# arkCyber/whisper-rust

Measured on AMD Instinct MI355X. Metric: real-time factor (audio-sec/wall-sec), greedy, 30 s synthetic chunks, higher is better.
Workload: dtype f16 operands / f32 accumulate; 1 GPU; ggml-small-shaped synthetic F16 model, greedy best_of=1 temperature_inc=0, 1 x 30 s 16 kHz f32 chunk per GPU, PCM resident in HBM; flash_attn=False, parallelism=chunk-dp1

## Files before the change

include/whisper_amd.h:

```cpp
#ifndef WHISPER_AMD_H
#define WHISPER_AMD_H

#include <stdbool.h>
#include <stddef.h>
#include <stdint.h>

#if defined(__GNUC__)
#  define WHISPER_API __attribute__((visibility("default")))
#else
#  define WHISPER_API
#endif

#define WHISPER_SAMPLE_RATE 16000
#define WHISPER_N_FFT       400
#define WHISPER_HOP_LENGTH  160
#define WHISPER_CHUNK_SIZE  30

#ifdef __cplusplus
extern "C" {
#endif

enum ggml_log_level {
    GGML_LOG_LEVEL_NONE  = 0,
    GGML_LOG_LEVEL_DEBUG = 1,
// ... 302 lines not shown
WHISPER_API struct whisper_vad_context_params whisper_vad_default_context_params(void);
WHISPER_API struct whisper_vad_context * whisper_vad_init_from_file_with_params(const char * path_model, struct whisper_vad_context_params params);
WHISPER_API struct whisper_vad_context * whisper_vad_init_with_params          (struct whisper_model_loader * loader, struct whisper_vad_context_params params);
WHISPER_API bool    whisper_vad_detect_speech(struct whisper_vad_context * vctx, const float * samples, int n_samples);
WHISPER_API int     whisper_vad_n_probs(struct whisper_vad_context * vctx);
WHISPER_API float * whisper_vad_probs  (struct whisper_vad_context * vctx);
WHISPER_API struct whisper_vad_segments * whisper_vad_segments_from_probs  (struct whisper_vad_context * vctx, struct whisper_vad_params params);
WHISPER_API struct whisper_vad_segments * whisper_vad_segments_from_samples(struct whisper_vad_context * vctx, struct whisper_vad_params params, const float * samples, int n_samples);
WHISPER_API int   whisper_vad_segments_n_segments(struct whisper_vad_segments * segments);
WHISPER_API float whisper_vad_segments_get_segment_t0(struct whisper_vad_segments * segments, int i_segment);
WHISPER_API float whisper_vad_segments_get_segment_t1(struct whisper_vad_segments * segments, int i_segment);
WHISPER_API void  whisper_vad_free_segments(struct whisper_vad_segments * segments);
WHISPER_API void  whisper_vad_free         (struct whisper_vad_context  * ctx);

WHISPER_API int          whisper_bench_memcpy          (int n_threads);
WHISPER_API const char * whisper_bench_memcpy_str      (int n_threads);
WHISPER_API int          whisper_bench_ggml_mul_mat    (int n_threads);
WHISPER_API const char * whisper_bench_ggml_mul_mat_str(int n_threads);


WHISPER_API void whisper_amd_abi_sizes(size_t out[6]);

WHISPER_API int64_t whisper_amd_get_mel      (struct whisper_state * state, float * dst, int64_t cap, int * n_len, int * n_mel);
WHISPER_API int64_t whisper_amd_get_embd_enc (struct whisper_state * state, float * dst, int64_t cap);
WHISPER_API int64_t whisper_amd_get_embd_conv(struct whisper_state * state, float * dst, int64_t cap);

WHISPER_API int64_t whisper_amd_vad_front  (struct whisper_vad_context * vctx, const float * samples, int n_samples, float * dst, int64_t cap);
WHISPER_API int     whisper_amd_vad_tile   (void);
WHISPER_API void    whisper_amd_vad_timings(struct whisper_vad_context * vctx, int64_t out_us[3]);

WHISPER_API void whisper_amd_get_timings_us(struct whisper_state * state, int64_t out[12]);
WHISPER_API void whisper_amd_reset_timings (struct whisper_state * state);

WHISPER_API void whisper_amd_gelu_table_f16(uint16_t * dst);

WHISPER_API void * whisper_amd_state_stream(struct whisper_state * state);

WHISPER_API int whisper_amd_decoder_info(struct whisper_state * state, int j, double out[8], int32_t * ids, int max_ids);

WHISPER_API int whisper_amd_decode_step_probe(struct whisper_context * ctx, struct whisper_state * state, int n_past, int n_iters, float * ms_per_step);

WHISPER_API int whisper_amd_mega_enabled(struct whisper_state * state);
WHISPER_API void whisper_amd_mega_role_of(int n_wg, int n_head, int wg, int * role, int * index);

WHISPER_API void whisper_amd_overlap_stats(struct whisper_state * state, int out[2]);

WHISPER_API int whisper_amd_mega_debug(struct whisper_context * ctx, struct whisper_state * state, int token, int n_past,
                                       unsigned long long * granules_out, float * logits_out);
WHISPER_API int whisper_amd_seq_debug(struct whisper_context * ctx, struct whisper_state * state, int token, int n_past, unsigned * values_out,
                                      float * logits_out);

WHISPER_API void whisper_amd_rows_stats(struct whisper_state * state, long out[2]);
WHISPER_API int  whisper_amd_rows_enabled(struct whisper_state * state);
WHISPER_API int whisper_amd_rows_debug(struct whisper_context * ctx, struct whisper_state * state, int B, int token, int n_past,
                                       unsigned long long * granules_out, float * logits_out);
WHISPER_API int whisper_amd_rows_step_probe(struct whisper_context * ctx, struct whisper_state ** states, int B, int n_past, int n_iters, float * ms_per_step);

WHISPER_API int whisper_amd_full_batch(struct whisper_context * ctx, struct whisper_state ** states, int n_chunks,
                                       struct whisper_full_params params, const float * const * samples, const int * n_samples);
WHISPER_API void whisper_amd_batch_stats(struct whisper_context * ctx, long * steps, long * rows);
WHISPER_API long whisper_amd_batch_one_launch(struct whisper_context * ctx);

#ifdef __cplusplus
}
#endif
#endif
// ... 1 lines not shown
```

whisper-rust_amd/csrc/wa_api.cpp:

```cpp
#include "wa_internal.h"

#include <algorithm>
#include <chrono>
#include <cmath>
#include <cstdarg>
#include <cstring>
#include <regex>
#include <thread>

static void wa_log_default(ggml_log_level, const char * text, void *) { fputs(text, stderr); fflush(stderr); }
static ggml_log_callback g_log_cb = wa_log_default;
static void * g_log_ud = nullptr;

void wa_log(ggml_log_level level, const char * fmt, ...) {
    if (!g_log_cb) return;
    char buf[1024];
    va_list ap;
    va_start(ap, fmt);
    const int n = vsnprintf(buf, sizeof(buf), fmt, ap);
    va_end(ap);
    if (n < (int) sizeof(buf)) { g_log_cb(level, buf, g_log_ud); return; }
    std::vector<char> big(n + 1);
    va_start(ap, fmt);
    vsnprintf(big.data(), big.size(), fmt, ap);
// ... 639 lines not shown
whisper_token_data whisper_full_get_token_data(struct whisper_context * ctx, int i, int j) { return ctx->state->result_all[i].tokens[j]; }
float whisper_full_get_token_p_from_state(struct whisper_state * st, int i, int j) { return st->result_all[i].tokens[j].p; }
float whisper_full_get_token_p(struct whisper_context * ctx, int i, int j) { return ctx->state->result_all[i].tokens[j].p; }
float whisper_full_get_segment_no_speech_prob_from_state(struct whisper_state * st, int i) { return st->result_all[i].no_speech_prob; }
float whisper_full_get_segment_no_speech_prob(struct whisper_context * ctx, int i) { return ctx->state->result_all[i].no_speech_prob; }

int          whisper_bench_memcpy(int) { return 0; }
const char * whisper_bench_memcpy_str(int) { return "whisper_bench_memcpy: not applicable to the HIP backend (use bench.py)\n"; }
int          whisper_bench_ggml_mul_mat(int) { return 0; }
const char * whisper_bench_ggml_mul_mat_str(int) { return "whisper_bench_ggml_mul_mat: not applicable to the HIP backend (use bench.py)\n"; }

static int64_t copy_out(whisper_state * st, const float * d_src, int64_t n, float * dst, int64_t cap) {
    if (!d_src) return -1;
    if (dst && cap > 0) {
        (void) hipSetDevice(st->ctx->device);
        (void) hipStreamSynchronize(st->stream);
        if (hipMemcpy(dst, d_src, (size_t) std::min(n, cap) * sizeof(float), hipMemcpyDeviceToHost) != hipSuccess) return -1;
    }
    return n;
}
int64_t whisper_amd_get_mel(struct whisper_state * st, float * dst, int64_t cap, int * n_len, int * n_mel) {
    if (n_len) *n_len = st->mel_n_len;
    if (n_mel) *n_mel = st->mel_n_mel;
    return copy_out(st, st->d_mel, (int64_t) st->mel_n_len * st->mel_n_mel, dst, cap);
}
int64_t whisper_amd_get_embd_enc(struct whisper_state * st, float * dst, int64_t cap) {
    if (!st->have_enc) return -1;
    return copy_out(st, st->d_embd_enc, (int64_t) st->enc_n_ctx * st->ctx->model.hp.n_audio_state, dst, cap);
}
int64_t whisper_amd_get_embd_conv(struct whisper_state * st, float * dst, int64_t cap) {
    if (!st->have_enc) return -1;
    return copy_out(st, st->d_embd_conv, (int64_t) st->enc_n_ctx * st->ctx->model.hp.n_audio_state, dst, cap);
}
void whisper_amd_gelu_table_f16(uint16_t * dst) {
    for (int i = 0; i < 65536; ++i) {
        _Float16 h; uint16_t u = (uint16_t) i; memcpy(&h, &u, 2);
        const float x = (float) h;
        const float g = 0.5f * x * (1.0f + tanhf(0.79788456080286535587989211986876f * x * (1.0f + 0.044715f * x * x)));
        _Float16 o = (_Float16) g; memcpy(&dst[i], &o, 2);
    }
}
void * whisper_amd_state_stream(struct whisper_state * st) { return (void *) st->stream; }

int whisper_amd_decoder_info(struct whisper_state * st, int j, double out[8], int32_t * ids, int max_ids) {
    if (!st || j < 0 || j >= WA_MAX_DECODERS) return -1;
    const auto & d = st->decoders[j];
    out[0] = d.failed; out[1] = d.completed; out[2] = d.has_ts; out[3] = d.seek_delta; out[4] = d.sequence.result_len;
    out[5] = d.sequence.avg_logprobs; out[6] = d.sequence.entropy; out[7] = st->no_speech_prob;
    const int n = (int) d.sequence.tokens.size();
    for (int i = 0; i < n && i < max_ids; ++i) ids[i] = d.sequence.tokens[i].id;
    return n;
}

int whisper_amd_full_batch(struct whisper_context * ctx, struct whisper_state ** states, int n_chunks, struct whisper_full_params params,
                           const float * const * samples, const int * n_samples) {
    if (!ctx || !states || n_chunks <= 0) return -1;
    std::vector<int> rc(n_chunks, 0);
    std::vector<std::thread> th;
    th.reserve(n_chunks);
    {
        wa_batch_groups groups(ctx, std::vector<whisper_state *>(states, states + n_chunks));
        for (int i = 0; i < n_chunks; ++i)
            th.emplace_back([&, i]() {
                rc[i] = whisper_full_with_state(ctx, states[i], params, samples[i], n_samples[i]);
                wa_batcher_leave(states[i]->batcher);
            });
// ... 8 lines not shown
```

whisper-rust_amd/csrc/wa_encode.cpp:

```cpp
#include "wa_internal.h"
#include "wa_kernels.h"
#include "wa_mega.h"
#include "wa_rows.h"

#include <algorithm>
#include <cmath>
#include <cstdlib>
#include <cstring>

template <typename T> static bool dev_alloc(T *& p, size_t n_elem, bool zero = true) {
    p = nullptr;
    const size_t bytes = n_elem * sizeof(T);
    if (!WA_HIP_OK(hipMalloc((void **) &p, bytes ? bytes : 256))) return false;
    if (zero && bytes) return WA_HIP_OK(hipMemset(p, 0, bytes));
    return true;
}
template <typename T> static void dev_free(T *& p) { if (p) { (void) hipFree(p); p = nullptr; } }

bool wa_kv_self_realloc(whisper_context & ctx, whisper_state & st, int n_cells) {
    const auto & hp = ctx.model.hp;
    if (n_cells > WA_ATT_MAXKV) { WA_ERROR("%s: %d KV cells exceed the attention kernels' limit (%d)\n", __func__, n_cells, WA_ATT_MAXKV); return false; }
    if (st.dec_graph) { (void) hipGraphExecDestroy(st.dec_graph); st.dec_graph = nullptr; }
    dev_free(st.kv_self.k);
    dev_free(st.kv_self.v);
    st.kv_self.size = n_cells;
    st.kv_self.head = 0;
    st.kv_self.n = 0;
    st.kv_self.cells.assign(n_cells, wa_kv_cell());
    const size_t n = (size_t) hp.n_text_layer * n_cells * hp.n_text_state;
    if (!dev_alloc(st.kv_self.k, n) || !dev_alloc(st.kv_self.v, n)) return false;
    dev_free(st.d_mask);
    st.d_mask_cap = (size_t) st.dec_mpad * n_cells;
    if (!dev_alloc(st.d_mask, st.d_mask_cap)) return false;
    if (st.h_stage_mask) { (void) hipHostFree(st.h_stage_mask); st.h_stage_mask = nullptr; }
    st.h_mask_cap = st.d_mask_cap;
    if (!WA_HIP_OK(hipHostMalloc((void **) &st.h_stage_mask, st.h_mask_cap))) return false;
    return true;
}

bool wa_rows_prepare(whisper_context & ctx, whisper_state & st) {
    if (!st.rows_form.enabled()) return false;
    if (st.d_rows_gr) return true;
    const auto & hp = ctx.model.hp;
    const int dt = hp.n_text_state, Ht = hp.n_text_head;
    const size_t row_gr = (size_t) 2 * dt;
    if (!dev_alloc(st.d_rows_gr, (size_t) hp.n_text_layer * WA_MEGA_EDGES * WA_ROWS_MAX * row_gr) ||
        !dev_alloc(st.d_rows_cgr, (size_t) hp.n_text_layer * WA_ROWS_MAX * Ht * WA_ROWS_CGR) || !dev_alloc(st.d_rows_status, 32)) {
        dev_free(st.d_rows_gr); dev_free(st.d_rows_cgr); dev_free(st.d_rows_status);
        st.rows_form.disable();
        return false;
    }
    return true;
}

bool wa_state_alloc(whisper_context & ctx, whisper_state & st) {
    const auto & hp = ctx.model.hp;
    const int d = hp.n_audio_state;
    st.ctx = &ctx;
    if (!WA_HIP_OK(hipSetDevice(ctx.device))) return false;
    if (!WA_HIP_OK(hipStreamCreateWithFlags(&st.stream, hipStreamNonBlocking))) return false;

    const int T = hp.n_audio_ctx, tpad = wa_pad(T, WA_TPAD);
    st.enc_tpad = tpad;
    st.cross_tpad = tpad;
    if (!dev_alloc(st.d_mel_max, 1)) return false;
    if (!dev_alloc(st.d_melT, (size_t) (2 * T + 8) * hp.n_mels + 512)) return false;
    if (!dev_alloc(st.d_h1,   (size_t) (2 * T + 8) * d)) return false;
    if (!dev_alloc(st.d_x,    (size_t) tpad * d)) return false;
    if (!dev_alloc(st.d_xn,   (size_t) tpad * d)) return false;
    if (!dev_alloc(st.d_qk,   (size_t) tpad * 2 * d)) return false;
    if (!dev_alloc(st.d_vt,   (size_t) d * tpad)) return false;
    if ((ctx.exact || ctx.model.wtype != 1) && hp.n_audio_state == hp.n_audio_head * 64)
        if (!dev_alloc(st.d_attn_p, (size_t) hp.n_audio_head * tpad * tpad) || !dev_alloc(st.d_attn_pl, (size_t) hp.n_audio_head * tpad * 32)) return false;
    if (!dev_alloc(st.d_ao,   (size_t) tpad * d)) return false;
    if (!dev_alloc(st.d_ff,   (size_t) tpad * 4 * d)) return false;
    if (!dev_alloc(st.d_embd_enc,  (size_t) tpad * d)) return false;
    if (!dev_alloc(st.d_embd_conv, (size_t) tpad * d)) return false;
    const size_t n_cross = (size_t) hp.n_text_layer * hp.n_text_head * tpad * 64;
    if (!dev_alloc(st.d_cross_k, n_cross) || !dev_alloc(st.d_cross_v, n_cross)) return false;

    const int mpad = wa_pad(hp.n_text_ctx, 64);
    st.dec_mpad = mpad;
    if (!dev_alloc(st.d_tok, mpad) || !dev_alloc(st.d_pos, mpad) || !dev_alloc(st.d_cell, mpad) || !dev_alloc(st.d_rows, mpad)) return false;
    if (!dev_alloc(st.d_dx,   (size_t) mpad * d)) return false;
    if (!dev_alloc(st.d_dxn,  (size_t) mpad * d)) return false;
    if (!dev_alloc(st.d_dqkv, (size_t) mpad * 3 * d)) return false;
    if (!dev_alloc(st.d_dao,  (size_t) mpad * d)) return false;
    if (!dev_alloc(st.d_dff,  (size_t) mpad * 4 * d)) return false;
    if (!dev_alloc(st.d_dq,   (size_t) mpad * d)) return false;
    if (!dev_alloc(st.d_logits, (size_t) WA_MAX_DECODERS * hp.n_vocab + 64, false)) return false;
    if (!dev_alloc(st.d_dyn, 8)) return false;
    { const char * g = getenv("WHISPER_AMD_NO_GRAPH"); st.graphs_enabled = !(g && g[0] == '1'); }
    {
        const char * g = getenv("WHISPER_AMD_NO_MEGA");
        const int dt = hp.n_text_state, Ht = hp.n_text_head;
        st.mega_form = wa_launch_form(!(g && g[0] == '1') && ctx.model.d_mega_layers && ctx.model.n_loaded > 0 && dt == Ht * 64 && dt % 128 == 0 &&
                                      dt <= WA_MEGA_MAX_D && hp.n_audio_ctx <= 1500 && ctx.model.n_cu >= 5 * Ht + 16 && tpad <= WA_MEGA_MAX_T &&
                                      !wa_wtype_has_min(ctx.model.wtype));
        if (st.mega_form.enabled()) {
            if (!dev_alloc(st.d_mega_cgr, (size_t) hp.n_text_layer * Ht * WA_MEGA_CGR)) return false;
            if (!dev_alloc(st.d_mega_gr, (size_t) hp.n_text_layer * WA_MEGA_EDGES * 4 * dt) || !dev_alloc(st.d_mega_out, (size_t) hp.n_vocab + 64)) return false;
            st.d_mega_status = (unsigned *) (st.d_mega_out + hp.n_vocab);
            if (!dev_alloc(st.d_mega_out2, (size_t) hp.n_vocab + 64) || !dev_alloc(st.d_mega_smask, (size_t) hp.n_vocab / 32 + 2)) return false;
            for (int b = 0; b < 2; ++b)
                if (!dev_alloc(st.d_mega_rec[b], (size_t) 512 * 8) || !dev_alloc(st.d_mega_ps[b], 8)) return false;
            {
// ... 134 lines not shown
    const int tpad = st.enc_tpad;
    hipStream_t s = st.stream;
    st.enc_n_ctx = T;

    const int rows_total = 2 * T + 8;
    wa_launch_mel_window(s, st.d_mel, hp.n_mels, st.mel_n_len, mel_offset, 2 * T, st.d_melT, rows_total);

    const bool exact = ctx.exact || m.wtype != 1;
    auto gemm = [&](wa_epi_mode mode, const wa_f16 * A, int lda, const wa_f16 * W, int ldw, int M, int N, int K, const wa_epi & e) {
        if (exact) wa_launch_gemm_exact(s, mode, A, lda, W, ldw, M, N, K, e);
        else       wa_launch_gemm(s, mode, A, lda, W, ldw, M, N, K, e);
    };

    {
        wa_epi e; e.bias = m.conv1.b; e.gelu = m.d_gelu; e.out = st.d_h1 + d; e.ldo = d;
        if (exact) {
            wa_launch_im2col3(s, st.d_melT, hp.n_mels, 0, 1, hp.n_mels, 2 * T, st.d_im2col, 3 * hp.n_mels);
            wa_launch_gemm_exact(s, WA_EPI_GELU_F16, st.d_im2col, 3 * hp.n_mels, m.conv1_g, 3 * hp.n_mels, 2 * T, d, 3 * hp.n_mels, e);
        } else {
            wa_launch_gemm(s, WA_EPI_GELU_F16, st.d_melT, hp.n_mels, m.conv1.w, m.conv1_kpad, 2 * T, d, m.conv1_kpad, e);
        }
    }
    {
        wa_epi e; e.bias = m.conv2.b; e.gelu = m.d_gelu; e.out = st.d_x; e.ldo = d; e.resid = m.e_pe; e.ldr = d; e.dbg = st.d_embd_conv;
        if (exact) {
            wa_launch_im2col3(s, st.d_h1, d, 0, 2, d, T, st.d_im2col, 3 * d);
            wa_launch_gemm_exact(s, WA_EPI_CONV2, st.d_im2col, 3 * d, m.conv2_g, 3 * d, T, d, 3 * d, e);
        } else {
            wa_launch_gemm(s, WA_EPI_CONV2, st.d_h1, 2 * d, m.conv2.w, 3 * d, T, d, 3 * d, e);
        }
    }

    const float KQscale = 1.0f / sqrtf(float(64));
    if (m.wtype != 1) {
        auto qmul = [&](wa_epi_mode mode, const wa_lin & L, int M, const wa_epi & e) {
            wa_launch_qgemm_exact(s, mode, st.d_q8, st.d_q8d, M, L.qs, L.qd, L.n_out, L.n_in, e, st.d_q8s, L.qm);
        };
        auto qlin = [&](wa_epi_mode mode, const float * A, int lda, const wa_lin & L, int M, const wa_epi & e) {
            wa_launch_quantize_q8_0(s, A, lda, M, L.n_in, st.d_q8, st.d_q8d, st.d_q8s);
            qmul(mode, L, M, e);
        };
        for (int il = 0; il < hp.n_audio_layer; ++il) {
            const auto & L = m.enc[il];
            wa_launch_layernorm_exact(s, st.d_x, d, T, d, L.attn_ln.w, L.attn_ln.b, hp.eps, nullptr, 0, nullptr, 0, st.d_q8, st.d_q8d, st.d_q8s);
            static const bool no_mfma_attn = getenv("WHISPER_AMD_NO_EXACT_MFMA") != nullptr;
            if (st.d_attn_p && T >= 128 && !no_mfma_attn) {
                { wa_epi e; e.bias = L.qkv.b; e.out = st.d_qk; e.ldo = 2 * d; e.out2 = st.d_vt; e.ldo2 = tpad; e.split0 = 2 * d; qmul(WA_EPI_ENC_QKV, L.qkv, T, e); }
                wa_launch_attn_exact_mfma(s, st.d_qk, 2 * d, st.d_vt, tpad, T, d, H, KQscale, st.d_attn_p, st.d_attn_pl, (T + 127) & ~127, st.d_ao, d, st.d_q32a);
                wa_launch_quantize_q8_0(s, st.d_q32a, d, T, d, st.d_q8, st.d_q8d, st.d_q8s);
            } else {
            { wa_epi e; e.bias = L.qkv.b; e.out = st.d_ff; e.ldo = 3 * d; qmul(WA_EPI_F16, L.qkv, T, e); }
            wa_launch_attn_exact(s, st.d_ff, 3 * d, st.d_ff + d, 64, 3 * d, st.d_ff + 2 * d, 64, 3 * d, H, T, T, nullptr, KQscale,
                                 st.d_att_partial, st.d_att_pleft, st.d_ao, d, nullptr, nullptr, nullptr, wa_q8_rows{ st.d_q8, st.d_q8d, st.d_q8s });
            }
            { wa_epi e; e.bias = L.out.b; e.out = st.d_x; e.ldo = d; e.resid = st.d_x; e.ldr = d; qmul(WA_EPI_RESID, L.out, T, e); }
            wa_launch_layernorm_exact(s, st.d_x, d, T, d, L.mlp_ln.w, L.mlp_ln.b, hp.eps, nullptr, 0, nullptr, 0, st.d_q8, st.d_q8d, st.d_q8s);
            { wa_epi e; e.bias = L.fc1.b; e.gelu = m.d_gelu; e.out = st.d_q32b; e.ldo = 4 * d; qmul(WA_EPI_GELU_F32, L.fc1, T, e); }
            { wa_epi e; e.bias = L.fc2.b; e.out = st.d_x; e.ldo = d; e.resid = st.d_x; e.ldr = d; qlin(WA_EPI_RESID, st.d_q32b, 4 * d, L.fc2, T, e); }
        }
        wa_launch_layernorm_exact(s, st.d_x, d, T, d, m.e_ln.w, m.e_ln.b, hp.eps, nullptr, 0, st.d_embd_enc, d);
        {
            wa_epi e; e.bias = m.cross_kv.b; e.scale = m.cross_kv.s; e.out = st.d_cross_k; e.out2 = st.d_cross_v; e.aux0 = st.cross_tpad; e.aux1 = d;
            qlin(WA_EPI_CROSS_KV, st.d_embd_enc, d, m.cross_kv, T, e);
        }
    } else {
    for (int il = 0; il < hp.n_audio_layer; ++il) {
        const auto & L = m.enc[il];
        if (exact) wa_launch_layernorm_exact(s, st.d_x, d, T, d, L.attn_ln.w, L.attn_ln.b, hp.eps, st.d_xn, d, nullptr, 0);
        else       wa_launch_layernorm(s, st.d_x, d, T, d, L.attn_ln.w, L.attn_ln.b, hp.eps, st.d_xn, d, nullptr, 0);
        static const bool no_mfma_attn = getenv("WHISPER_AMD_NO_EXACT_MFMA") != nullptr;
        if (exact && st.d_attn_p && T >= 128 && !no_mfma_attn) {
            wa_epi e; e.bias = L.qkv.b; e.out = st.d_qk; e.ldo = 2 * d; e.out2 = st.d_vt; e.ldo2 = tpad; e.split0 = 2 * d;
            wa_launch_gemm_exact(s, WA_EPI_ENC_QKV, st.d_xn, d, L.qkv.w, d, T, 3 * d, d, e);
            wa_launch_attn_exact_mfma(s, st.d_qk, 2 * d, st.d_vt, tpad, T, d, H, KQscale, st.d_attn_p, st.d_attn_pl, (T + 127) & ~127, st.d_ao, d);
        } else if (exact) {
            wa_epi e; e.bias = L.qkv.b; e.out = st.d_ff; e.ldo = 3 * d;
            wa_launch_gemm_exact(s, WA_EPI_F16, st.d_xn, d, L.qkv.w, d, T, 3 * d, d, e);
            wa_launch_attn_exact(s, st.d_ff, 3 * d, st.d_ff + d, 64, 3 * d, st.d_ff + 2 * d, 64, 3 * d, H, T, T, nullptr, KQscale,
                                 st.d_att_partial, st.d_att_pleft, st.d_ao, d, nullptr);
        } else {
            wa_epi e; e.bias = L.qkv.b; e.out = st.d_qk; e.ldo = 2 * d; e.out2 = st.d_vt; e.ldo2 = tpad; e.split0 = 2 * d;
            wa_launch_gemm(s, WA_EPI_ENC_QKV, st.d_xn, d, L.qkv.w, d, T, 3 * d, d, e);
            wa_launch_enc_attn(s, st.d_qk, 2 * d, st.d_vt, tpad, T, d, H, KQscale, st.d_ao, d);
        }
        {
            wa_epi e; e.bias = L.out.b; e.out = st.d_x; e.ldo = d; e.resid = st.d_x; e.ldr = d;
            gemm(WA_EPI_RESID, st.d_ao, d, L.out.w, d, T, d, d, e);
        }
        if (exact) wa_launch_layernorm_exact(s, st.d_x, d, T, d, L.mlp_ln.w, L.mlp_ln.b, hp.eps, st.d_xn, d, nullptr, 0);
        else       wa_launch_layernorm(s, st.d_x, d, T, d, L.mlp_ln.w, L.mlp_ln.b, hp.eps, st.d_xn, d, nullptr, 0);
        {
            wa_epi e; e.bias = L.fc1.b; e.gelu = m.d_gelu; e.out = st.d_ff; e.ldo = 4 * d;
            gemm(WA_EPI_GELU_F16, st.d_xn, d, L.fc1.w, d, T, 4 * d, d, e);
        }
        {
            wa_epi e; e.bias = L.fc2.b; e.out = st.d_x; e.ldo = d; e.resid = st.d_x; e.ldr = d;
            gemm(WA_EPI_RESID, st.d_ff, 4 * d, L.fc2.w, 4 * d, T, d, 4 * d, e);
        }
    }
    if (exact) wa_launch_layernorm_exact(s, st.d_x, d, T, d, m.e_ln.w, m.e_ln.b, hp.eps, st.d_xn, d, st.d_embd_enc, d);
    else       wa_launch_layernorm(s, st.d_x, d, T, d, m.e_ln.w, m.e_ln.b, hp.eps, st.d_xn, d, st.d_embd_enc, d);

    {
        wa_epi e; e.bias = m.cross_kv.b; e.scale = m.cross_kv.s; e.out = st.d_cross_k; e.out2 = st.d_cross_v; e.aux0 = st.cross_tpad; e.aux1 = d;
        gemm(WA_EPI_CROSS_KV, st.d_xn, d, m.cross_kv.w, d, T, hp.n_text_layer * 2 * d, d, e);
    }
    }
// ... 7 lines not shown
```

whisper-rust_amd/csrc/wa_exact.hip:

```cpp
#include "wa_device.h"
#include <cstdlib>

#define EX_LD 40

template <int EPI>
__global__ __launch_bounds__(256, 2) void k_gemm_exact(const wa_f16 * __restrict__ A, int lda, const wa_f16 * __restrict__ W, int ldw,
                                                       int M, int N, int K, wa_epi e) {
    __shared__ __attribute__((aligned(16))) wa_f16 As[2][32 * EX_LD];
    __shared__ __attribute__((aligned(16))) wa_f16 Ws[2][32 * EX_LD];
    const int tid = threadIdx.x, lane = tid & 63, wave = tid >> 6;
    const int wm = wave >> 1, wn = wave & 1, li = lane >> 3, lj = lane & 7;
    const int tiles_n = (N + 31) / 32;
    const int m0 = (blockIdx.x / tiles_n) * 32, n0 = (blockIdx.x % tiles_n) * 32;

    float acc[2][2][32];
#pragma unroll
    for (int p = 0; p < 2; ++p)
#pragma unroll
        for (int q = 0; q < 2; ++q)
#pragma unroll
            for (int i = 0; i < 32; ++i) acc[p][q][i] = 0.0f;

    const int np = K & ~31, nsteps = np >> 5;
    const int lrow = (tid & 127) >> 2, lkc = tid & 3;
// ... 893 lines not shown
    float inv;
    {
        const double delta = 2.0 * (double) (ng + 8) * 0x1p-53 * tot * 1.000001;
        const float ilo = (float) (1.0 / (tot + delta)), ihi = (float) (1.0 / (tot - delta));
        inv = ilo;
        if (ilo != ihi) {
            double sum = 0.0;
            if (u == 0) {
                for (int g = 0; g < ng; ++g) { const float * v = srow + 8 * g; sum += (double) (((v[0] + v[4]) + (v[2] + v[6])) + ((v[1] + v[5]) + (v[3] + v[7]))); }
                for (int c = n8; c < T; ++c) sum += (double) srow[c];
            }
            sum = __shfl(sum, lane & ~31, WAVE);
            inv = (float) (1.0 / sum);
        }
    }
    if (jq >= T) return;
    wa_f16 * prow = P + ((size_t) h * T + jq) * kvp;
    wa_f16 * plrow = p_left + ((size_t) h * T + jq) * 32;
    typedef unsigned as_u4 __attribute__((ext_vector_type(4)));
    for (int g = u; g < (kvp >> 3); g += LPR) {
        as_u4 pk = { 0u, 0u, 0u, 0u };
        const int c0 = 8 * g;
        if (c0 < np) {
            const float4 lo = *(const float4 *) (srow + c0), hi = *(const float4 *) (srow + c0 + 4);
            pk.x = (unsigned) f2h(lo.x * inv) | ((unsigned) f2h(lo.y * inv) << 16); pk.y = (unsigned) f2h(lo.z * inv) | ((unsigned) f2h(lo.w * inv) << 16);
            pk.z = (unsigned) f2h(hi.x * inv) | ((unsigned) f2h(hi.y * inv) << 16); pk.w = (unsigned) f2h(hi.z * inv) | ((unsigned) f2h(hi.w * inv) << 16);
        } else {
            for (int c = c0; c < c0 + 8 && c < T; ++c) plrow[c - np] = f2h(srow[c] * inv);
        }
        *(as_u4 *) (prow + c0) = pk;
    }
}

void wa_launch_attn_exact_mfma(hipStream_t s, const wa_f16 * qk, int ldqk, const wa_f16 * vt, int ldvt, int T, int d, int n_head, float scale,
                               wa_f16 * p, wa_f16 * p_left, int kvp, wa_f16 * out, int ldo, float * out32) {
    static bool attr_done = false;
    const int lds = AS_Q * (kvp + AS_PAD) * (int) sizeof(float);
    if (!attr_done) { (void) hipFuncSetAttribute((const void *) k_attn_scores_mfma, hipFuncAttributeMaxDynamicSharedMemorySize, 160 * 1024 - 4096); attr_done = true; }
    hipLaunchKernelGGL(k_attn_scores_mfma, dim3(n_head, (T + AS_Q - 1) / AS_Q), dim3(AS_THREADS), lds, s, qk, ldqk, d, T, scale, p, p_left, kvp);
    const int np = T & ~31;
    wa_epi e; e.out = out; e.ldo = ldo; e.out2 = p_left; e.bs_o2 = (long long) T * 32; e.aux0 = np; e.aux1 = T - np;
    e.out3 = out32; e.ldo3 = ldo;
    e.bs_a = (long long) T * kvp; e.bs_w = (long long) 64 * ldvt;
    gemm_exact_mfma_launch<WA_EPI_ATTN_PV>(s, p, kvp, vt, ldvt, T, 64, (np + 127) & ~127, e, n_head);
}

template <int NQ>
__global__ __launch_bounds__(ATT_THREADS) void k_attn_exact_mq(const wa_f16 * __restrict__ q, int ldq, const wa_f16 * __restrict__ kbase, size_t k_head_stride,
                                                               int k_row_stride, const wa_f16 * __restrict__ vbase, size_t v_head_stride, int v_row_stride,
                                                               int n_tokens, int n_kv, int kvp, const int8_t * __restrict__ mask, float scale,
                                                               wa_f16 * __restrict__ out, int ldo, float * __restrict__ qk_out,
                                                               float * __restrict__ out32, int8_t * __restrict__ q8, float * __restrict__ q8d, float * __restrict__ q8s) {
    constexpr int NW = ATT_THREADS / 64;
    extern __shared__ __attribute__((aligned(16))) unsigned char mq_smem[];
    float  * sc   = (float *) mq_smem;
    float  * gs   = sc + (size_t) NQ * kvp;
    float  * part = gs + (size_t) NQ * (kvp >> 3);
    wa_f16 * p16  = (wa_f16 *) (part + (size_t) NQ * 32 * 64);
    __shared__ float red[NQ][NW];
    __shared__ double redd[NQ][NW];
    __shared__ float s_inv[NQ];
    __shared__ __attribute__((aligned(16))) wa_f16 qs[NQ][64];

    const int tid = threadIdx.x, lane = tid & 63, wave = tid >> 6;
    const int n_head = gridDim.x;
    const int h = blockIdx.x, j0 = blockIdx.y * NQ;
    const wa_f16 * kp = kbase + (size_t) h * k_head_stride;
    const wa_f16 * vp = vbase + (size_t) h * v_head_stride;
// ... 225 lines not shown
```

whisper-rust_amd/csrc/wa_internal.h:

```cpp
#pragma once

#include "../../include/whisper_amd.h"
#include "wa_one_launch.h"
#include "wa_grammar.h"
#include "wa_vad.h"

#include <hip/hip_runtime.h>

#include <cstdint>
#include <cstdio>
#include <map>
#include <memory>
#include <mutex>
#include <random>
#include <set>
#include <string>
#include <atomic>
#include <vector>

#define WA_MAX_DECODERS 8
#define WA_TPAD         128

void wa_log(ggml_log_level level, const char * fmt, ...) __attribute__((format(printf, 2, 3)));
#define WA_INFO(...)  wa_log(GGML_LOG_LEVEL_INFO,  __VA_ARGS__)
// ... 137 lines not shown
};

struct wa_decoder {
    wa_sequence sequence;
    int  i_batch = 0, seek_delta = 0;
    bool failed = false, completed = false, has_ts = false;
    std::vector<float> probs, logits, logprobs;
    std::vector<std::pair<double, int>> logits_id;
    mutable std::mt19937 rng;
    wa_grammar_state grammar;
    wa_grammar_cache grammar_cache;
};

struct whisper_state {
    whisper_context * ctx = nullptr;
    hipStream_t stream = nullptr;

    int64_t t_sample_us = 0, t_encode_us = 0, t_decode_us = 0, t_batchd_us = 0, t_prompt_us = 0, t_mel_us = 0;
    int32_t n_sample = 0, n_encode = 0, n_decode = 0, n_batchd = 0, n_prompt = 0, n_fail_p = 0, n_fail_h = 0;

    int mel_n_len = 0, mel_n_len_org = 0, mel_n_mel = 0;
    float * d_mel = nullptr; size_t d_mel_cap = 0;
    float * d_pcm = nullptr; size_t d_pcm_cap = 0;
    unsigned int * d_mel_max = nullptr;

    int enc_n_ctx = 0;
    int enc_tpad  = 0;
    wa_f16 * d_melT   = nullptr;
    wa_f16 * d_h1     = nullptr;
    float  * d_x      = nullptr;
    wa_f16 * d_xn     = nullptr;
    wa_f16 * d_qk     = nullptr;
    wa_f16 * d_vt     = nullptr;
    wa_f16 * d_attn_p = nullptr;
    wa_f16 * d_attn_pl = nullptr;
    wa_f16 * d_ao     = nullptr;
    wa_f16 * d_ff     = nullptr;
    float  * d_embd_enc  = nullptr;
    float  * d_embd_conv = nullptr;
    bool     have_enc = false;

    wa_f16 * d_cross_k = nullptr, * d_cross_v = nullptr;
    int cross_tpad = 0;

    wa_kv_cache kv_self;
    int kv_self_n_dec = 0;

    int dec_mpad = 0;
    int32_t * d_tok = nullptr, * d_pos = nullptr, * d_cell = nullptr;
    int8_t  * d_mask = nullptr; size_t d_mask_cap = 0;
    float  * d_dx  = nullptr;
    wa_f16 * d_dxn = nullptr;
    wa_f16 * d_dqkv = nullptr;
    wa_f16 * d_dao = nullptr;
    wa_f16 * d_dff = nullptr;
    wa_f16 * d_dq  = nullptr;
    float  * d_att_partial = nullptr;
    wa_f16 * d_att_pleft = nullptr;
    wa_f16 * d_im2col = nullptr;
    float  * d_logits = nullptr;
    int32_t * d_rows = nullptr;
    float  * d_aheads_qk = nullptr;
    float  * d_q32a = nullptr;
    float  * d_q32b = nullptr;
    int8_t * d_q8   = nullptr;
    int      q8_rows = 0;
    float  * d_q8d  = nullptr;
    float  * d_q8s  = nullptr;
// ... 94 lines not shown
```

whisper-rust_amd/csrc/wa_kernels.h:

```cpp
#pragma once
#include <hip/hip_runtime.h>
#include <cstdint>

typedef uint16_t wa_f16;

#define WA_ATT_MAXKV 5120

enum wa_epi_mode {
    WA_EPI_F16 = 0,
    WA_EPI_ENC_QKV,
    WA_EPI_GELU_F16,
    WA_EPI_RESID,
    WA_EPI_CONV2,
    WA_EPI_F32,
    WA_EPI_CROSS_KV,
    WA_EPI_GELU_F32,
    WA_EPI_DEC_QKV,
    WA_EPI_ATTN_PV,
};

struct wa_rowptr { wa_f16 * kv_k; wa_f16 * kv_v; const wa_f16 * cross_k; const wa_f16 * cross_v; int n_kv; int kv_head; };

struct wa_q8_rows { int8_t * qs = nullptr; float * qd = nullptr; float * qsum = nullptr; };

// ... 12 lines not shown
    const int * dyn = nullptr;
    long long bs_a = 0, bs_w = 0, bs_o2 = 0;
    const wa_rowptr * rowp = nullptr; long long rowp_off = 0;
};

void wa_launch_gemm(hipStream_t stream, wa_epi_mode mode, const wa_f16 * A, int lda, const wa_f16 * W, int ldw,
                    int M, int N, int K, const wa_epi & e);

void wa_launch_mel(hipStream_t stream, const float * pcm, int n_samples, const float * hann, const float * sincos,
                   const float * filters, int n_mel, int n_fft_bins, float * mel, int n_len, unsigned int * mel_max);

void wa_launch_mel_window(hipStream_t stream, const float * mel, int n_mel, int n_len, int seek, int n_frames,
                          wa_f16 * melT, int rows_total);

void wa_launch_layernorm(hipStream_t stream, const float * x, int ldx, int rows, int d, const float * w, const float * b,
                         float eps, wa_f16 * out16, int ld16, float * out32, int ld32);

void wa_launch_enc_attn(hipStream_t stream, const wa_f16 * qk, int ldqk, const wa_f16 * vt, int ldvt, int T, int d,
                        int n_head, float scale, wa_f16 * out, int ldo);

void wa_launch_dec_embed(hipStream_t stream, const int32_t * tok, const int32_t * pos, int n_tokens, int d,
                         const wa_f16 * te, const float * pe, float * x);

void wa_launch_gemm_exact(hipStream_t stream, wa_epi_mode mode, const wa_f16 * A, int lda, const wa_f16 * W, int ldw, int M, int N, int K,
                          const wa_epi & e);
void wa_launch_gemv_exact(hipStream_t stream, wa_epi_mode mode, const wa_f16 * A, int lda, const int32_t * rows, const wa_f16 * W, int ldw,
                          int M, int N, int K, const wa_epi & e);
void wa_launch_ln_gemv_exact(hipStream_t stream, wa_epi_mode mode, const float * x, int ldx, const int32_t * rows, const float * ln_w,
                             const float * ln_b, float eps, const wa_f16 * W, int ldw, int M, int N, int K, const wa_epi & e);
void wa_launch_im2col3(hipStream_t stream, const wa_f16 * src, int src_ld, int row0, int stride, int IC, int OL, wa_f16 * dst, int dst_ld);
void wa_launch_layernorm_exact(hipStream_t stream, const float * x, int ldx, int rows, int d, const float * w, const float * b, float eps,
                               wa_f16 * out16, int ld16, float * out32, int ld32, int8_t * qs = nullptr, float * qd = nullptr,
                               float * qsum = nullptr );
void wa_launch_attn_exact_mfma(hipStream_t stream, const wa_f16 * qk, int ldqk, const wa_f16 * vt, int ldvt, int T, int d, int n_head, float scale,
                               wa_f16 * p, wa_f16 * p_left, int kvp, wa_f16 * out, int ldo,
                               float * out32 = nullptr );
void wa_launch_attn_exact(hipStream_t stream, const wa_f16 * q, int ldq, const wa_f16 * kbase, size_t k_head_stride, int k_row_stride,
                          const wa_f16 * vbase, size_t v_head_stride, int v_row_stride, int n_head, int n_tokens, int n_kv, const int8_t * mask,
                          float scale, float * partial, wa_f16 * p_left, wa_f16 * out, int ldo, float * qk_out, const int * dyn_n_kv = nullptr,
                          float * out32 = nullptr ,
                          wa_q8_rows q8 = wa_q8_rows() ,
                          const wa_rowptr * rowp = nullptr, int rowp_cross = 0, long long rowp_off = 0
                          );

void wa_launch_quantize_q8_0(hipStream_t stream, const float * x, int ldx, int rows, int K, int8_t * qs, float * qd, float * qsum = nullptr);
void wa_launch_qgemm_exact(hipStream_t stream, wa_epi_mode mode, const int8_t * xq, const float * xd, int M, const int8_t * wq, const float * wd, int N, int K,
                           const wa_epi & e, const float * xs = nullptr, const float * wm = nullptr);
void wa_launch_ln_q8_row(hipStream_t stream, const float * x, int K, const float * w, const float * b, float eps, int8_t * qs, float * qd, float * qsum = nullptr);
void wa_launch_qgemv_gelu_q8(hipStream_t stream, const int8_t * xq, const float * xd, const int8_t * wq, const float * wd, int N, int K, const float * bias,
                             const wa_f16 * gelu, int8_t * oq, float * oqd, const float * xs = nullptr, const float * wm = nullptr, float * oqs = nullptr);
void wa_launch_dec_embed_q(hipStream_t stream, const int32_t * tok, const int32_t * pos, int n_tokens, int d, const int8_t * wq, const float * wd,
                           const float * pe, float * x, const float * wm = nullptr);
```

Before: 360.0 x real-time.

## Fuse exact encoder attention scores, softmax and PV into one kernel

Adds a fused exact-attention kernel that computes QK scores, softmax and the P·V product per head and query tile inside LDS. This removes the HBM round-trip of the probability matrix and the second kernel launch. The P buffers are now allocated lazily, only when the two-kernel path is forced or the scores do not fit in LDS. The large LDS footprint (about 100KB at T=1500) may limit occupancy, and the summation order has to stay bit-exact.

```diff
diff --git a/include/whisper_amd.h b/include/whisper_amd.h
--- a/include/whisper_amd.h
+++ b/include/whisper_amd.h
@@ -358,6 +358,8 @@
 WHISPER_API void whisper_amd_get_timings_us(struct whisper_state * state, int64_t out[12]);
 WHISPER_API void whisper_amd_reset_timings (struct whisper_state * state);
 
+WHISPER_API void whisper_amd_enc_attn_stats(struct whisper_state * state, long out[3]);
+
 WHISPER_API void whisper_amd_gelu_table_f16(uint16_t * dst);
 
 WHISPER_API void * whisper_amd_state_stream(struct whisper_state * state);
diff --git a/whisper-rust_amd/csrc/wa_api.cpp b/whisper-rust_amd/csrc/wa_api.cpp
--- a/whisper-rust_amd/csrc/wa_api.cpp
+++ b/whisper-rust_amd/csrc/wa_api.cpp
@@ -695,6 +695,11 @@
     if (!st->have_enc) return -1;
     return copy_out(st, st->d_embd_conv, (int64_t) st->enc_n_ctx * st->ctx->model.hp.n_audio_state, dst, cap);
 }
+void whisper_amd_enc_attn_stats(struct whisper_state * st, long out[3]) {
+    out[0] = st->n_attn_fused; out[1] = st->n_attn_two;
+    const size_t H = st->ctx->model.hp.n_audio_head, tpad = st->enc_tpad;
+    out[2] = (long) (((st->d_attn_p ? H * tpad * tpad : 0) + (st->d_attn_pl ? H * tpad * 32 : 0)) * sizeof(wa_f16));
+}
 void whisper_amd_gelu_table_f16(uint16_t * dst) {
     for (int i = 0; i < 65536; ++i) {
         _Float16 h; uint16_t u = (uint16_t) i; memcpy(&h, &u, 2);
diff --git a/whisper-rust_amd/csrc/wa_encode.cpp b/whisper-rust_amd/csrc/wa_encode.cpp
--- a/whisper-rust_amd/csrc/wa_encode.cpp
+++ b/whisper-rust_amd/csrc/wa_encode.cpp
@@ -53,6 +53,12 @@
     return true;
 }
 
+static bool wa_attn_p_ensure(whisper_state & st) {
+    if (st.d_attn_p && st.d_attn_pl) return true;
+    const size_t H = st.ctx->model.hp.n_audio_head, tpad = st.enc_tpad;
+    return dev_alloc(st.d_attn_p, H * tpad * tpad) && dev_alloc(st.d_attn_pl, H * tpad * 32);
+}
+
 bool wa_state_alloc(whisper_context & ctx, whisper_state & st) {
     const auto & hp = ctx.model.hp;
     const int d = hp.n_audio_state;
@@ -70,8 +76,7 @@
     if (!dev_alloc(st.d_xn,   (size_t) tpad * d)) return false;
     if (!dev_alloc(st.d_qk,   (size_t) tpad * 2 * d)) return false;
     if (!dev_alloc(st.d_vt,   (size_t) d * tpad)) return false;
-    if ((ctx.exact || ctx.model.wtype != 1) && hp.n_audio_state == hp.n_audio_head * 64)
-        if (!dev_alloc(st.d_attn_p, (size_t) hp.n_audio_head * tpad * tpad) || !dev_alloc(st.d_attn_pl, (size_t) hp.n_audio_head * tpad * 32)) return false;
+    st.attn_mfma = (ctx.exact || ctx.model.wtype != 1) && hp.n_audio_state == hp.n_audio_head * 64;
     if (!dev_alloc(st.d_ao,   (size_t) tpad * d)) return false;
     if (!dev_alloc(st.d_ff,   (size_t) tpad * 4 * d)) return false;
     if (!dev_alloc(st.d_embd_enc,  (size_t) tpad * d)) return false;
@@ -272,6 +277,17 @@
     }
 
     const float KQscale = 1.0f / sqrtf(float(64));
+    static const bool no_mfma_attn = getenv("WHISPER_AMD_NO_EXACT_MFMA") != nullptr;
+    const int attn_kvp = (T + 127) & ~127;
+    const bool attn_mfma = exact && st.attn_mfma && T >= 128 && !no_mfma_attn;
+    bool attn_two = false;
+    if (attn_mfma) {
+        const char * g = getenv("WHISPER_AMD_ATTN_TWO_KERNELS");
+        attn_two = (g && g[0] == '1') || !wa_attn_exact_fused_fits(attn_kvp);
+        if (attn_two && !wa_attn_p_ensure(st)) return false;
+        (attn_two ? st.n_attn_two : st.n_attn_fused) += hp.n_audio_layer;
+    }
+    wa_f16 * const attn_p = attn_two ? st.d_attn_p : nullptr, * const attn_pl = attn_two ? st.d_attn_pl : nullptr;
     if (m.wtype != 1) {
         auto qmul = [&](wa_epi_mode mode, const wa_lin & L, int M, const wa_epi & e) {
             wa_launch_qgemm_exact(s, mode, st.d_q8, st.d_q8d, M, L.qs, L.qd, L.n_out, L.n_in, e, st.d_q8s, L.qm);
@@ -283,10 +299,9 @@
         for (int il = 0; il < hp.n_audio_layer; ++il) {
             const auto & L = m.enc[il];
             wa_launch_layernorm_exact(s, st.d_x, d, T, d, L.attn_ln.w, L.attn_ln.b, hp.eps, nullptr, 0, nullptr, 0, st.d_q8, st.d_q8d, st.d_q8s);
-            static const bool no_mfma_attn = getenv("WHISPER_AMD_NO_EXACT_MFMA") != nullptr;
-            if (st.d_attn_p && T >= 128 && !no_mfma_attn) {
+            if (attn_mfma) {
                 { wa_epi e; e.bias = L.qkv.b; e.out = st.d_qk; e.ldo = 2 * d; e.out2 = st.d_vt; e.ldo2 = tpad; e.split0 = 2 * d; qmul(WA_EPI_ENC_QKV, L.qkv, T, e); }
-                wa_launch_attn_exact_mfma(s, st.d_qk, 2 * d, st.d_vt, tpad, T, d, H, KQscale, st.d_attn_p, st.d_attn_pl, (T + 127) & ~127, st.d_ao, d, st.d_q32a);
+                wa_launch_attn_exact_mfma(s, st.d_qk, 2 * d, st.d_vt, tpad, T, d, H, KQscale, attn_p, attn_pl, attn_kvp, st.d_ao, d, st.d_q32a);
                 wa_launch_quantize_q8_0(s, st.d_q32a, d, T, d, st.d_q8, st.d_q8d, st.d_q8s);
             } else {
             { wa_epi e; e.bias = L.qkv.b; e.out = st.d_ff; e.ldo = 3 * d; qmul(WA_EPI_F16, L.qkv, T, e); }
@@ -308,11 +323,10 @@
         const auto & L = m.enc[il];
         if (exact) wa_launch_layernorm_exact(s, st.d_x, d, T, d, L.attn_ln.w, L.attn_ln.b, hp.eps, st.d_xn, d, nullptr, 0);
         else       wa_launch_layernorm(s, st.d_x, d, T, d, L.attn_ln.w, L.attn_ln.b, hp.eps, st.d_xn, d, nullptr, 0);
-        static const bool no_mfma_attn = getenv("WHISPER_AMD_NO_EXACT_MFMA") != nullptr;
-        if (exact && st.d_attn_p && T >= 128 && !no_mfma_attn) {
+        if (attn_mfma) {
             wa_epi e; e.bias = L.qkv.b; e.out = st.d_qk; e.ldo = 2 * d; e.out2 = st.d_vt; e.ldo2 = tpad; e.split0 = 2 * d;
             wa_launch_gemm_exact(s, WA_EPI_ENC_QKV, st.d_xn, d, L.qkv.w, d, T, 3 * d, d, e);
-            wa_launch_attn_exact_mfma(s, st.d_qk, 2 * d, st.d_vt, tpad, T, d, H, KQscale, st.d_attn_p, st.d_attn_pl, (T + 127) & ~127, st.d_ao, d);
+            wa_launch_attn_exact_mfma(s, st.d_qk, 2 * d, st.d_vt, tpad, T, d, H, KQscale, attn_p, attn_pl, attn_kvp, st.d_ao, d);
         } else if (exact) {
             wa_epi e; e.bias = L.qkv.b; e.out = st.d_ff; e.ldo = 3 * d;
             wa_launch_gemm_exact(s, WA_EPI_F16, st.d_xn, d, L.qkv.w, d, T, 3 * d, d, e);
diff --git a/whisper-rust_amd/csrc/wa_exact.hip b/whisper-rust_amd/csrc/wa_exact.hip
--- a/whisper-rust_amd/csrc/wa_exact.hip
+++ b/whisper-rust_amd/csrc/wa_exact.hip
@@ -949,8 +949,218 @@
     }
 }
 
+#ifndef AS_KDEPTH
+#define AS_KDEPTH 2
+#endif
+#define AF_VDEPTH 4
+#define AF_MERGE_BYTES (4 * 8 * 64 * 16)
+
+__global__ __launch_bounds__(AS_THREADS) void k_attn_exact_fused(const wa_f16 * __restrict__ qk, int ldqk, int d, int T, float scale,
+                                                                 const wa_f16 * __restrict__ vt, int ldvt, int kvp,
+                                                                 wa_f16 * __restrict__ out, int ldo, float * __restrict__ out32) {
+    extern __shared__ __attribute__((aligned(16))) unsigned char as_smem[];
+    float * sc = (float *) as_smem;
+    const int kvs = kvp + AS_PAD;
+    f32x4 * mg = (f32x4 *) (as_smem + (size_t) AS_Q * kvs * sizeof(float));
+    __shared__ float red[AS_THREADS / 64][AS_Q];
+    __shared__ __attribute__((aligned(16))) wa_f16 pls[AS_Q][32];
+    const int tid = threadIdx.x, lane = tid & 63, wave = __builtin_amdgcn_readfirstlane(tid >> 6);
+    const int h = blockIdx.x, j0 = blockIdx.y * AS_Q;
+    const int fr = lane & 15, fb = lane >> 4;
+
+    float qf[2][8];
+    {
+        const wa_f16 * qrow = qk + (size_t) min(j0 + fr, T - 1) * ldqk + h * 64 + 8 * fb;
+#pragma unroll
+        for (int st = 0; st < 2; ++st) {
+            const half8 v = *(const half8 *) (qrow + 32 * st);
+#pragma unroll
+            for (int i = 0; i < 8; ++i) qf[st][i] = (float) v[i];
+        }
+    }
+    const wa_f16 * kcol = qk + d + h * 64 + 8 * fb;
+    const int ntiles = (T + 15) >> 4;
+    constexpr int NWV = AS_THREADS / 64;
+    float lmax[4] = { -INFINITY, -INFINITY, -INFINITY, -INFINITY };
+    half8 kn[AS_KDEPTH][2];
+#pragma unroll
+    for (int s = 0; s < AS_KDEPTH; ++s) {
+        const wa_f16 * kr = kcol + (size_t) min((wave + NWV * s) * 16 + fr, T - 1) * ldqk;
+        kn[s][0] = *(const half8 *) kr; kn[s][1] = *(const half8 *) (kr + 32);
+    }
+    for (int kb = wave; kb < ntiles; kb += NWV * AS_KDEPTH) {
+#pragma unroll
+        for (int s = 0; s < AS_KDEPTH; ++s) {
+            const int kt = kb + NWV * s;
+            if (kt >= ntiles) break;
+            const half8 k0 = kn[s][0], k1 = kn[s][1];
+            {
+                const wa_f16 * kr = kcol + (size_t) min((kt + NWV * AS_KDEPTH) * 16 + fr, T - 1) * ldqk;
+                kn[s][0] = *(const half8 *) kr; kn[s][1] = *(const half8 *) (kr + 32);
+            }
+            as_f16v acc[8];
+            const as_f16v zero = { 0.f, 0.f, 0.f, 0.f, 0.f, 0.f, 0.f, 0.f, 0.f, 0.f, 0.f, 0.f, 0.f, 0.f, 0.f, 0.f };
+#pragma unroll
+            for (int i = 0; i < 8; ++i) acc[i] = __builtin_amdgcn_mfma_f32_16x16x1f32(qf[0][i], (float) k0[i], zero, 0, 0, 0);
+#pragma unroll
+            for (int i = 0; i < 8; ++i) acc[i] = __builtin_amdgcn_mfma_f32_16x16x1f32(qf[1][i], (float) k1[i], acc[i], 0, 0, 0);
+            const int key = kt * 16 + fr;
+            f32x4 a[8];
+#pragma unroll
+            for (int i = 0; i < 8; ++i) {
+                const f32x4 b0 = __builtin_shufflevector(acc[i], acc[i], 0, 1, 2, 3), b1 = __builtin_shufflevector(acc[i], acc[i], 4, 5, 6, 7);
+                const f32x4 b2 = __builtin_shufflevector(acc[i], acc[i], 8, 9, 10, 11), b3 = __builtin_shufflevector(acc[i], acc[i], 12, 13, 14, 15);
+                a[i] = (b0 + b2) + (b1 + b3);
+            }
+            const f32x4 t0 = a[0] + a[4], t1 = a[1] + a[5], t2 = a[2] + a[6], t3 = a[3] + a[7];
+            const f32x4 r4 = ((t0 + t1) + (t2 + t3)) * scale;
+#pragma unroll
+            for (int j = 0; j < 4; ++j)
+                if (key < T) { sc[(size_t) (4 * fb + j) * kvs + key] = r4[j]; lmax[j] = fmaxf(lmax[j], r4[j]); }
+        }
+    }
+#pragma unroll
+    for (int j = 0; j < 4; ++j) {
+        float m = lmax[j];
+        m = fmaxf(m, dpp_f32<0x128>(m)); m = fmaxf(m, dpp_f32<0x124>(m)); m = fmaxf(m, dpp_f32<0x122>(m)); m = fmaxf(m, dpp_f32<0x121>(m));
+        if (fr == 0) red[wave][4 * fb + j] = m;
+    }
+    __syncthreads();
+
+    constexpr int LPR = AS_THREADS / AS_Q;
+    const int row = tid / LPR, u = tid % LPR;
+    float * srow = sc + (size_t) row * kvs;
+    float mx = red[0][row];
+#pragma unroll
+    for (int w = 1; w < NWV; ++w) mx = fmaxf(mx, red[w][row]);
+    const int n8 = T & ~7, ng = n8 >> 3, np = T & ~31, kpv = (np + 127) & ~127, nk = kpv >> 7;
+    double ps = 0.0;
+    for (int g = u; g < ng; g += LPR) {
+        float4 lo = *(const float4 *) (srow + 8 * g), hi = *(const float4 *) (srow + 8 * g + 4);
+        lo.x = wa_expf(lo.x - mx); lo.y = wa_expf(lo.y - mx); lo.z = wa_expf(lo.z - mx); lo.w = wa_expf(lo.w - mx);
+        hi.x = wa_expf(hi.x - mx); hi.y = wa_expf(hi.y - mx); hi.z = wa_expf(hi.z - mx); hi.w = wa_expf(hi.w - mx);
+        *(float4 *) (srow + 8 * g) = lo; *(float4 *) (srow + 8 * g + 4) = hi;
+        ps += (double) (((lo.x + hi.x) + (lo.z + hi.z)) + ((lo.y + hi.y) + (lo.w + hi.w)));
+    }
+    for (int c = n8 + u; c < T; c += LPR) { const float ev = wa_expf_libm(srow[c] - mx); srow[c] = ev; ps += (double) ev; }
+    ps += dpp_f64<0x111>(ps); ps += dpp_f64<0x112>(ps); ps += dpp_f64<0x114>(ps); ps += dpp_f64<0x118>(ps);
+    ps += dpp_f64<0x142, 0xa>(ps);
+    double tot = __shfl(ps, lane | 31, WAVE);
+    asm volatile("s_waitcnt lgkmcnt(0)" ::: "memory");
+    float inv;
+    {
+        const double delta = 2.0 * (double) (ng + 8) * 0x1p-53 * tot * 1.000001;
+        const float ilo = (float) (1.0 / (tot + delta)), ihi = (float) (1.0 / (tot - delta));
+        inv = ilo;
+        if (ilo != ihi) {
+            double sum = 0.0;
+            if (u == 0) {
+                for (int g = 0; g < ng; ++g) { const float * v = srow + 8 * g; sum += (double) (((v[0] + v[4]) + (v[2] + v[6])) + ((v[1] + v[5]) + (v[3] + v[7]))); }
+                for (int c = n8; c < T; ++c) sum += (double) srow[c];
+            }
+            sum = __shfl(sum, lane & ~31, WAVE);
+            inv = (float) (1.0 / sum);
+        }
+    }
+
+    const int ct = wave & 3, hf = wave >> 2, fk = fb;
+    const wa_f16 * vrow = vt + (size_t) (h * 64 + ct * 16 + fr) * ldvt;
+    const wa_f16 * vfrag = vrow + 32 * fk + 8 * hf;
+    half8 vr[AF_VDEPTH][2];
+#pragma unroll
+    for (int s = 0; s < AF_VDEPTH; ++s) {
+        const wa_f16 * v = vfrag + 128 * min(s, nk - 1);
+        vr[s][0] = *(const half8 *) v; vr[s][1] = *(const half8 *) (v + 16);
+    }
+
+    typedef unsigned as_u4 __attribute__((ext_vector_type(4)));
+    { const int c = np + u; pls[row][u] = c < T ? f2h(srow[c] * inv) : (wa_f16) 0; }
+    asm volatile("" ::: "memory");
+    unsigned char * brow = (unsigned char *) srow;
+    for (int g = u; g < (kpv >> 3); g += LPR) {
+        as_u4 pk = { 0u, 0u, 0u, 0u };
+        const int c0 = 8 * g;
+        if (c0 < np) {
+            const float4 lo = *(const float4 *) (srow + c0), hi = *(const float4 *) (srow + c0 + 4);
+            pk.x = (unsigned) f2h(lo.x * inv) | ((unsigned) f2h(lo.y * inv) << 16); pk.y = (unsigned) f2h(lo.z * inv) | ((unsigned) f2h(lo.w * inv) << 16);
+            pk.z = (unsigned) f2h(hi.x * inv) | ((unsigned) f2h(hi.y * inv) << 16); pk.w = (unsigned) f2h(hi.z * inv) | ((unsigned) f2h(hi.w * inv) << 16);
+        }
+        asm volatile("" ::: "memory");
+        *(as_u4 *) (brow + 16 * g) = pk;
+        asm volatile("" ::: "memory");
+    }
+    wa_barrier_lds();
+
+    f32x4 acc[16];
+#pragma unroll
+    for (int r = 0; r < 16; ++r) acc[r] = (f32x4){0.f, 0.f, 0.f, 0.f};
+    const wa_f16 * pfrag = (const wa_f16 *) (sc + (size_t) fr * kvs) + 32 * fk + 8 * hf;
+    for (int kb = 0; kb < nk; kb += AF_VDEPTH) {
+#pragma unroll
+        for (int s = 0; s < AF_VDEPTH; ++s) {
+            const int kt = kb + s;
+            if (kt >= nk) break;
+            const half8 v0 = vr[s][0], v1 = vr[s][1];
+            {
+                const wa_f16 * v = vfrag + 128 * min(kt + AF_VDEPTH, nk - 1);
+                vr[s][0] = *(const half8 *) v; vr[s][1] = *(const half8 *) (v + 16);
+            }
+            const half8 p0 = *(const half8 *) (pfrag + 128 * kt), p1 = *(const half8 *) (pfrag + 128 * kt + 16);
+#pragma unroll
+            for (int i = 0; i < 8; ++i) acc[i] = __builtin_amdgcn_mfma_f32_16x16x4f32((float) p0[i], (float) v0[i], acc[i], 0, 0, 0);
+#pragma unroll
+            for (int i = 0; i < 8; ++i) acc[8 + i] = __builtin_amdgcn_mfma_f32_16x16x4f32((float) p1[i], (float) v1[i], acc[8 + i], 0, 0, 0);
+        }
+    }
+    f32x4 uu[8];
+#pragma unroll
+    for (int l = 0; l < 8; ++l) uu[l] = acc[l] + acc[8 + l];
+    if (hf == 1) {
+#pragma unroll
+        for (int l = 0; l < 8; ++l) mg[(ct * 8 + l) * 64 + lane] = uu[l];
+    }
+    wa_barrier_lds();
+    if (hf == 1) return;
+    f32x4 a[8];
+#pragma unroll
+    for (int l = 0; l < 8; ++l) a[l] = uu[l] + mg[(ct * 8 + l) * 64 + lane];
+    const f32x4 t0 = a[0] + a[4], t1 = a[1] + a[5], t2 = a[2] + a[6], t3 = a[3] + a[7];
+    const f32x4 res = (t0 + t1) + (t2 + t3);
+
+    const int nl = T - np, on = h * 64 + ct * 16 + fr;
+    half8 vl[4];
+#pragma unroll
+    for (int c = 0; c < 4; ++c) vl[c] = nl > 0 ? *(const half8 *) (vrow + np + 8 * c) : (half8) (_Float16) 0;
+#pragma unroll
+    for (int j = 0; j < 4; ++j) {
+        const int m = 4 * fk + j;
+        half8 pv[4];
+#pragma unroll
+        for (int c = 0; c < 4; ++c) pv[c] = *(const half8 *) (&pls[m][8 * c]);
+        double sumf = (double) res[j];
+        float prod[32];
+#pragma unroll
+        for (int c = 0; c < 32; ++c) prod[c] = (float) vl[c >> 3][c & 7] * (float) pv[c >> 3][c & 7];
+#pragma unroll
+        for (int c = 0; c < 32; ++c) if (c < nl) sumf += (double) prod[c];
+        if (j0 + m < T) {
+            if (out32) out32[(size_t) (j0 + m) * ldo + on] = (float) sumf;
+            else out[(size_t) (j0 + m) * ldo + on] = f2h((float) sumf);
+        }
+    }
+}
+
+static int attn_fused_lds(int kvp) { return AS_Q * (kvp + AS_PAD) * (int) sizeof(float) + AF_MERGE_BYTES; }
+bool wa_attn_exact_fused_fits(int kvp) { return attn_fused_lds(kvp) <= 160 * 1024 - 4096; }
+
 void wa_launch_attn_exact_mfma(hipStream_t s, const wa_f16 * qk, int ldqk, const wa_f16 * vt, int ldvt, int T, int d, int n_head, float scale,
                                wa_f16 * p, wa_f16 * p_left, int kvp, wa_f16 * out, int ldo, float * out32) {
+    if (!p) {
+        static bool attr_done = false;
+        if (!attr_done) { (void) hipFuncSetAttribute((const void *) k_attn_exact_fused, hipFuncAttributeMaxDynamicSharedMemorySize, 160 * 1024 - 4096); attr_done = true; }
+        hipLaunchKernelGGL(k_attn_exact_fused, dim3(n_head, (T + AS_Q - 1) / AS_Q), dim3(AS_THREADS), attn_fused_lds(kvp), s, qk, ldqk, d, T, scale, vt, ldvt, kvp, out, ldo, out32);
+        return;
+    }
     static bool attr_done = false;
     const int lds = AS_Q * (kvp + AS_PAD) * (int) sizeof(float);
     if (!attr_done) { (void) hipFuncSetAttribute((const void *) k_attn_scores_mfma, hipFuncAttributeMaxDynamicSharedMemorySize, 160 * 1024 - 4096); attr_done = true; }
diff --git a/whisper-rust_amd/csrc/wa_internal.h b/whisper-rust_amd/csrc/wa_internal.h
--- a/whisper-rust_amd/csrc/wa_internal.h
+++ b/whisper-rust_amd/csrc/wa_internal.h
@@ -193,8 +193,10 @@
     wa_f16 * d_xn     = nullptr;
     wa_f16 * d_qk     = nullptr;
     wa_f16 * d_vt     = nullptr;
+    bool     attn_mfma = false;
     wa_f16 * d_attn_p = nullptr;
     wa_f16 * d_attn_pl = nullptr;
+    long     n_attn_fused = 0, n_attn_two = 0;
     wa_f16 * d_ao     = nullptr;
     wa_f16 * d_ff     = nullptr;
     float  * d_embd_enc  = nullptr;
diff --git a/whisper-rust_amd/csrc/wa_kernels.h b/whisper-rust_amd/csrc/wa_kernels.h
--- a/whisper-rust_amd/csrc/wa_kernels.h
+++ b/whisper-rust_amd/csrc/wa_kernels.h
@@ -68,6 +68,7 @@
 void wa_launch_layernorm_exact(hipStream_t stream, const float * x, int ldx, int rows, int d, const float * w, const float * b, float eps,
                                wa_f16 * out16, int ld16, float * out32, int ld32, int8_t * qs = nullptr, float * qd = nullptr,
                                float * qsum = nullptr );
+bool wa_attn_exact_fused_fits(int kvp);
 void wa_launch_attn_exact_mfma(hipStream_t stream, const wa_f16 * qk, int ldqk, const wa_f16 * vt, int ldvt, int T, int d, int n_head, float scale,
                                wa_f16 * p, wa_f16 * p_left, int kvp, wa_f16 * out, int ldo,
                                float * out32 = nullptr );
```

New measurement: 360.1 x real-time, median of 2. Within noise of the previous version (+0.0%).
